# Ignaciagothe/tda-eeg-audio

Measured on AMD Instinct MI355X. Metric: windows/sec end-to-end (dist->Rips H0/H1->Wasserstein), 47-ch EEG, higher is better.
Workload: dtype f64; 1 GPU; configs[4]+configs[2]: 1416 recordings x 5 bands x 15 selected windows = 106200 (EEG 47x250 f64, audio 250 f64) window pairs per pass, the whole job; per pair corr->dist->Rips H0/H1 (EEG 47 pts), tau per recording-band, Takens dim 3 sub 2 + Rips (audio, 23..123 pts over the bands), Wasserstein H0+H1, features, per-recording reductions; one all-gather of the (1416, 5x48) rows per pass; windows_per_pass=106200, windows_per_gpu_per_pass=106200, input_bytes_per_gpu=10195200000, batches_per_pass=1, windows_per_batch=106200, parallelism=recordings dealt over 1 rank(s), one all-gather per pass, batches_in_flight=3, hip_graph=True, batches_rerun_with_full_ladder=0

## Files before the change

include/tdaeeg.h:

```cpp
#ifndef TDAEEG_H
#define TDAEEG_H

#include <stddef.h>

#ifdef __cplusplus
extern "C" {
#endif

typedef struct tda_ctx tda_ctx;

typedef enum {
    TDA_OK = 0,
    TDA_ERR_INVALID = 1,
    TDA_ERR_HIP = 2,
    TDA_ERR_UNSUPPORTED = 3,
    TDA_ERR_NOMEM = 4
} tda_status;

#define TDA_WIN_OK            0
#define TDA_WIN_H1_TRUNCATED  1
#define TDA_WIN_CLASS_OVERFLOW 2
#define TDA_WIN_DEGENERATE    4
#define TDA_WIN_NOT_CONVERGED 8
#define TDA_WIN_TOO_LARGE     16
// ... 125 lines not shown
tda_status tda_tau_segments_dev(tda_ctx* ctx, const double* win, const int* seg_off, int n_seg, int n_t,
                                int max_lag, int* tau_seg, int* tau_win, void* stream);

tda_status tda_features_batch_dev(tda_ctx* ctx, const double* dgm, const int* cnt, int n_dgm,
                                  int cap, double* feat, void* stream);
tda_status tda_features_batch(tda_ctx* ctx, const double* dgm, const int* cnt, int n_dgm,
                              int cap, double* feat);

typedef struct {
    double* rows;
    const int* cnt;
    int cap;
    int order;
    double* feat;
} tda_diagram_set;
tda_status tda_diagram_finish_dev(tda_ctx* ctx, const tda_diagram_set* sets, int n_sets, int n_dgm, void* stream);
#define TDA_ORDER_IN_CALL  0
#define TDA_ORDER_DEFERRED 1
tda_status tda_set_h1_order(tda_ctx* ctx, int policy);
#define TDA_SCHEME_LISTS 0
#define TDA_SCHEME_GRID  1
#define TDA_SCHEME_ONE   2
tda_status tda_set_launch_scheme(tda_ctx* ctx, int scheme);

tda_status tda_aggregate_batch_dev(tda_ctx* ctx, const double* feat_h0, const double* feat_h1,
                                   const int* seg_off, int n_seg, double* out, void* stream);
tda_status tda_aggregate_batch(tda_ctx* ctx, const double* feat_h0, const double* feat_h1,
                               const int* seg_off, int n_seg, int n_total, double* out);

tda_status tda_segment_nanmean_dev(tda_ctx* ctx, const double* x, const int* seg_off, int n_seg,
                                   double* out, void* stream);
tda_status tda_segment_nanmean(tda_ctx* ctx, const double* x, const int* seg_off, int n_seg,
                               int n_total, double* out);

tda_status tda_recording_rows_dev(tda_ctx* ctx, const double* w_h0, const double* w_h1, const int* tau_seg,
                                  const double* feat_h0, const double* feat_h1, const int* seg_off,
                                  int n_seg, double* out, const int* status_a, const int* status_b,
                                  int* seg_flags, void* stream);

tda_status tda_spearman_batch_dev(tda_ctx* ctx, const double* x, const double* y, int ld, const int* cols,
                                  int n_cols, const int* seg_off, int n_seg, double* r, void* stream);
tda_status tda_spearman_batch(tda_ctx* ctx, const double* x, const double* y, int n_total, int ld,
                              const int* cols, int n_cols, const int* seg_off, int n_seg, double* r);

tda_status tda_temporal_corr_dev(tda_ctx* ctx, const double* fa, const double* fe, int ld, const int* cols,
                                 int n_cols, const int* seg_off, int n_seg, const int* status_b, double* out,
// ... 50 lines not shown
```

tda_eeg_audio_amd/_lib.py:

```python
import contextlib
import ctypes as C
import os

import numpy as np

_HERE = os.path.dirname(os.path.abspath(__file__))
LIB_PATH = os.path.join(_HERE, os.path.basename(os.environ.get("TDA_LIB", "libtdaeeg.so")))

c_dp = C.POINTER(C.c_double)
c_ip = C.POINTER(C.c_int)
c_vp = C.c_void_p

TDA_WIN_H1_TRUNCATED = 1
TDA_WIN_CLASS_OVERFLOW = 2
TDA_WIN_DEGENERATE = 4
TDA_WIN_NOT_CONVERGED = 8
TDA_WIN_TOO_LARGE = 16
TDA_WIN_NO_PAIR = 32
N_FEATURES = 11
MAX_POINTS = 128

_I, _D = C.c_int, C.c_double
SYMBOLS = {
    "tda_version": (_I, []),
# ... 23 lines not shown
    "tda_sosfiltfilt": (_I, [c_vp, c_vp, _I, _I, c_vp, c_vp, _I, _I, c_vp]),
    "tda_filtfilt_dev": (_I, [c_vp, c_vp, _I, _I, c_vp, c_vp, c_vp, _I, _I, c_vp, c_vp, c_vp]),
    "tda_filtfilt": (_I, [c_vp, c_vp, _I, _I, c_vp, c_vp, c_vp, _I, _I, c_vp]),
    "tda_sosfiltfilt_bank_dev": (_I, [c_vp, c_vp, _I, _I, c_vp, c_vp, _I, _I, _I, c_vp, c_vp, c_vp]),
    "tda_filtfilt_bank_dev": (_I, [c_vp, c_vp, _I, _I, c_vp, c_vp, c_vp, _I, _I, _I, c_vp, c_vp, c_vp]),
    "tda_sosfiltfilt_bank_ragged_dev": (_I, [c_vp, c_vp, _I, _I, c_vp, c_vp, c_vp, c_vp, c_vp, _I, _I, _I, c_vp, c_vp, c_vp]),
    "tda_filtfilt_bank_ragged_dev": (_I, [c_vp, c_vp, _I, c_vp, c_vp, c_vp, c_vp, c_vp, c_vp, _I, _I, _I, c_vp, c_vp, c_vp]),
    "tda_gather_windows_dev": (_I, [c_vp, c_vp, c_vp, _I, _I, c_vp, c_vp]),
    "tda_eeg_window_ragged_dev": (_I, [c_vp, c_vp, c_vp, c_vp, _I, _I, _I, _D, c_vp, c_vp, c_vp, _I, c_vp, c_vp, _I, c_vp,
                                       c_vp, c_vp]),
    "tda_upfirdn_dev": (_I, [c_vp, c_vp, C.c_longlong, c_vp, _I, _I, _I, C.c_longlong, C.c_longlong, c_vp, c_vp]),
    "tda_upfirdn": (_I, [c_vp, c_vp, C.c_longlong, c_vp, _I, _I, _I, C.c_longlong, C.c_longlong, c_vp]),
    "tda_hilbert_envelope_dev": (_I, [c_vp, c_vp, _I, c_vp, c_vp, c_vp]),
    "tda_hilbert_envelope": (_I, [c_vp, c_vp, _I, c_vp, c_vp]),
    "tda_resample_poly_ragged_dev": (_I, [c_vp, c_vp, _I, c_vp, c_vp, c_vp, c_vp, c_vp, _I, _I, _I, _I, c_vp, c_vp]),
    "tda_hilbert_envelope_ragged_dev": (_I, [c_vp, c_vp, _I, c_vp, c_vp, c_vp, c_vp, c_vp, c_vp, c_vp]),
    "tda_tau_batch_dev": (_I, [c_vp, c_vp, _I, _I, _I, c_vp, c_vp]),
    "tda_tau_segments_dev": (_I, [c_vp, c_vp, c_vp, _I, _I, _I, c_vp, c_vp, c_vp]),
    "tda_recording_rows_dev": (_I, [c_vp, c_vp, c_vp, c_vp, c_vp, c_vp, c_vp, _I, c_vp, c_vp, c_vp, c_vp, c_vp]),
    "tda_set_retry_policy": (_I, [c_vp, _I]),
    "tda_set_retry_counter": (_I, [c_vp, c_vp]),
    "tda_set_h1_order": (_I, [c_vp, _I]),
    "tda_set_launch_scheme": (_I, [c_vp, _I]),
    "tda_diagram_finish_dev": (_I, [c_vp, c_vp, _I, _I, c_vp]),
    "tda_tau_batch": (_I, [c_vp, c_vp, _I, _I, _I, c_vp]),
    "tda_features_batch_dev": (_I, [c_vp, c_vp, c_vp, _I, _I, c_vp, c_vp]),
    "tda_features_batch": (_I, [c_vp, c_vp, c_vp, _I, _I, c_vp]),
    "tda_aggregate_batch_dev": (_I, [c_vp, c_vp, c_vp, c_vp, _I, c_vp, c_vp]),
    "tda_aggregate_batch": (_I, [c_vp, c_vp, c_vp, c_vp, _I, _I, c_vp]),
    "tda_segment_nanmean_dev": (_I, [c_vp, c_vp, c_vp, _I, c_vp, c_vp]),
    "tda_segment_nanmean": (_I, [c_vp, c_vp, c_vp, _I, _I, c_vp]),
    "tda_spearman_batch_dev": (_I, [c_vp, c_vp, c_vp, _I, c_vp, _I, c_vp, _I, c_vp, c_vp]),
    "tda_spearman_batch": (_I, [c_vp, c_vp, c_vp, _I, _I, c_vp, _I, c_vp, _I, c_vp]),
    "tda_temporal_corr_dev": (_I, [c_vp, c_vp, c_vp, _I, c_vp, _I, c_vp, _I, c_vp, c_vp, c_vp]),
    "tda_temporal_corr_batch": (_I, [c_vp, c_vp, c_vp, _I, _I, c_vp, _I, c_vp, _I, c_vp, c_vp]),
    "tda_wasserstein_batch_dev": (_I, [c_vp, c_vp, c_vp, _I, c_vp, c_vp, _I, c_vp, c_vp, _I, c_vp, c_vp, c_vp]),
    "tda_wasserstein_cross_dev": (_I, [c_vp, c_vp, c_vp, _I, _I, c_vp, c_vp, _I, c_vp, c_vp, _I, _I, c_vp, _I, c_vp, c_vp,
                                       c_vp, c_vp, c_vp]),
    "tda_cross_rows_dev": (_I, [c_vp, c_vp, c_vp, c_vp, c_vp, c_vp, _I, c_vp, c_vp, c_vp, c_vp]),
    "tda_wasserstein_matrix_dev": (_I, [c_vp, c_vp, c_vp, _I, _I, c_vp, _I, c_vp, c_vp, c_vp, _I, _I, c_vp, _I, _I, c_vp,
                                        c_vp, c_vp, c_vp, c_vp]),
    "tda_match_rows_dev": (_I, [c_vp, c_vp, c_vp, c_vp, _I, _I, c_vp, c_vp, c_vp, c_vp, c_vp, c_vp]),
    "tda_wasserstein_batch": (_I, [c_vp, c_vp, c_vp, _I, _I, c_vp, c_vp, _I, _I, c_vp, c_vp, _I, c_vp, c_vp]),
    "tda_event_create": (_I, [c_vp, C.POINTER(c_vp)]),
    "tda_event_record": (_I, [c_vp, c_vp, c_vp]),
    "tda_event_elapsed_ms": (_I, [c_vp, c_vp, c_vp, C.POINTER(C.c_float)]),
# ... 68 lines not shown

    ORDER_IN_CALL, ORDER_DEFERRED = 0, 1

    def set_h1_order(self, policy):
        self.check(self.lib.tda_set_h1_order(self.h, int(policy)))

    @contextlib.contextmanager
    def deferred(self, retry="auto"):
        if retry != "auto":
            self.set_retry_policy(self.RETRY_FIRST_PASS if retry == "first" else self.RETRY_ONE_STEP)
        self.set_h1_order(self.ORDER_DEFERRED)
        try:
            yield self
        finally:
            self.set_h1_order(self.ORDER_IN_CALL)
            if retry != "auto":
                self.set_retry_policy(self.RETRY_AUTO)

    SCHEME_LISTS, SCHEME_GRID, SCHEME_ONE = 0, 1, 2

    def set_launch_scheme(self, scheme):
        self.check(self.lib.tda_set_launch_scheme(self.h, int(scheme)))

    def set_retry_counter(self, dev_ptr):
        self.check(self.lib.tda_set_retry_counter(self.h, c_vp(dev_ptr) if dev_ptr else None))

    PROBES = {"rips_audio": 1, "rips_eeg": 2, "corr_dist": 3}

    def new_event(self):
        ev = c_vp()
        self.check(self.lib.tda_event_create(self.h, C.byref(ev)))
        return ev

    def arm_probe(self, stage, ev_start=None, ev_stop=None, dev_span=None):
        self.check(self.lib.tda_set_kernel_probe(self.h, self.PROBES[stage], ev_start, ev_stop,
                                                 c_vp(dev_span) if dev_span else None))

    def elapsed_ms(self, ev_start, ev_stop):
        ms = C.c_float()
        self.check(self.lib.tda_event_elapsed_ms(self.h, ev_start, ev_stop, C.byref(ms)))
        return float(ms.value)

    def close(self):
        if getattr(self, "h", None):
            self.lib.tda_ctx_destroy(self.h)
            self.h = None
# ... 39 lines not shown
```

tda_eeg_audio_amd/csrc/capi.hip:

```cpp
#include "common.h"
#include <string.h>
#include <vector>

static thread_local std::string g_create_err;

#pragma GCC visibility push(default)
extern "C" {

int tda_version(void) { return 100; }

tda_status tda_ctx_create(int device_id, tda_ctx** out)
{
    if (!out) return TDA_ERR_INVALID;
    *out = nullptr;
    int ndev = 0;
    hipError_t e = hipGetDeviceCount(&ndev);
    if (e != hipSuccess || ndev <= 0) {
        g_create_err = std::string("no HIP device: ") + hipGetErrorString(e);
        return TDA_ERR_HIP;
    }
    if (device_id < 0 || device_id >= ndev) { g_create_err = "device_id out of range"; return TDA_ERR_INVALID; }
    e = hipSetDevice(device_id);
    if (e != hipSuccess) { g_create_err = std::string("hipSetDevice: ") + hipGetErrorString(e); return TDA_ERR_HIP; }
    tda_ctx* c = new (std::nothrow) tda_ctx();
// ... 31 lines not shown
{
    if (!ctx) return TDA_ERR_INVALID;
    if ((words_dm != 0 && words_dm != 1 && words_dm != 2 && words_dm != 4) || (words_cloud != 1 && words_cloud != 2))
        TDA_FAIL(ctx, TDA_ERR_INVALID, "class words: dm in {0,1,2,4}, cloud in {1,2}");
    ctx->words_dm = words_dm;
    ctx->words_cloud = words_cloud;
    return TDA_OK;
}

tda_status tda_set_h1_order(tda_ctx* ctx, int policy)
{
    if (!ctx) return TDA_ERR_INVALID;
    if (policy != TDA_ORDER_IN_CALL && policy != TDA_ORDER_DEFERRED) TDA_FAIL(ctx, TDA_ERR_INVALID, "unknown order policy");
    ctx->h1_order = policy;
    return TDA_OK;
}

tda_status tda_set_launch_scheme(tda_ctx* ctx, int scheme)
{
    if (!ctx) return TDA_ERR_INVALID;
    if (scheme != TDA_SCHEME_LISTS && scheme != TDA_SCHEME_GRID && scheme != TDA_SCHEME_ONE)
        TDA_FAIL(ctx, TDA_ERR_INVALID, "unknown launch scheme");
    ctx->launch_scheme = scheme;
    return TDA_OK;
}

tda_status tda_diagram_finish_dev(tda_ctx* ctx, const tda_diagram_set* sets, int n_sets, int n_dgm, void* stream)
{
    if (!ctx) return TDA_ERR_INVALID;
    if (n_dgm < 0) TDA_FAIL(ctx, TDA_ERR_INVALID, "negative count");
    if (n_sets && !sets) TDA_FAIL(ctx, TDA_ERR_INVALID, "null pointer");
    return launch_diagram_finish(ctx, sets, n_sets, n_dgm, (hipStream_t)stream);
}

tda_status tda_set_retry_counter(tda_ctx* ctx, void* dev_counters)
{
    if (!ctx) return TDA_ERR_INVALID;
    ctx->retry_ctr = (unsigned long long*)dev_counters;
    return TDA_OK;
}

tda_status tda_set_retry_policy(tda_ctx* ctx, int policy)
{
    if (!ctx) return TDA_ERR_INVALID;
    if (policy < TDA_RETRY_AUTO || policy > TDA_RETRY_LAST_RUNG) TDA_FAIL(ctx, TDA_ERR_INVALID, "unknown retry policy");
    ctx->retry_policy = policy;
// ... 780 lines not shown
```

tda_eeg_audio_amd/csrc/common.h:

```cpp
#pragma once
#include <hip/hip_runtime.h>
#include <stdint.h>
#include <string>
#include <vector>
#include "../../include/tdaeeg.h"

typedef unsigned long long u64;
typedef uint32_t u32;
typedef uint16_t u16;

struct tda_ctx {
    int device = 0;
    int words_dm = 2;
    int words_cloud = 1;
    int retry_policy = 0;
    unsigned long long* retry_ctr = nullptr;
    unsigned long long* total_scratch = nullptr;
    int h1_order = 0;
    int launch_scheme = 0;
    int* retry_buf[32] = {};
    int* fin_list[32] = {};
    int* ws_list[32] = {};
    hipStream_t retry_stream[32] = {};
    int retry_streams = 0;
    int retry_shared = 0;
    int retry_cap = 0;
    std::vector<void*> retired;
    void* ws = nullptr;
    size_t ws_bytes = 0;
    std::string err;
    struct Probe { hipEvent_t start = nullptr, stop = nullptr; unsigned long long* span = nullptr; bool armed = false; };
    Probe probe[4];
};

struct ProbeScope {
    tda_ctx* ctx; hipStream_t st; int which; bool on; unsigned long long* span;
    ProbeScope(tda_ctx* c, int w, hipStream_t s)
        : ctx(c), st(s), which(w), on(w > 0 && w < 4 && c->probe[w].armed), span(nullptr)
    {
        if (on) {
            span = ctx->probe[which].span;
            if (ctx->probe[which].start) (void)hipEventRecord(ctx->probe[which].start, st);
// ... 172 lines not shown
```

tda_eeg_audio_amd/csrc/wasserstein.hip:

```cpp
#include "common.h"
#include <type_traits>

#ifdef TDA_PROFILE
__device__ unsigned long long g_prof_ws[16];
extern "C" __attribute__((visibility("default"))) int tda_profile_read_ws(unsigned long long* out, int reset)
{
    if (hipMemcpyFromSymbol(out, HIP_SYMBOL(g_prof_ws), sizeof(unsigned long long) * 16) != hipSuccess) return 1;
    if (reset) {
        unsigned long long z[16] = {0};
        if (hipMemcpyToSymbol(HIP_SYMBOL(g_prof_ws), z, sizeof(z)) != hipSuccess) return 1;
    }
    return 0;
}
#define WPROF(i, v) do { if (lane_id() == 0) atomicAdd(&g_prof_ws[i], (unsigned long long)(v)); } while (0)
#define WCLK() clock64()
#else
#define WPROF(i, v) do {} while (0)
#define WCLK() 0ull
#endif

#define WS_DEFERRED 0x40000000
#define WS_CP 0.7071067811865476
#define WS_SP 0.7071067811865475

// ... 5 lines not shown
}

__device__ __forceinline__ double wave_min_f64_ws(double v)
{
#pragma unroll
    for (int off = 32; off > 0; off >>= 1) {
        const double o = __shfl_xor(v, off, 64);
        v = o < v ? o : v;
    }
    return v;
}

__device__ __forceinline__ double ws_cost(double ab, double ad, double bb, double bd)
{
    const double xx = ab * ab + ad * ad;
    const double yy = bb * bb + bd * bd;
    const double dot = fma(ad, bd, ab * bb);
    double d2 = -2.0 * dot;
    d2 += xx;
    d2 += yy;
    if (!(d2 > 0.0)) d2 = 0.0;
    return sqrt_rn(d2);
}

struct ws_index_pairs {
    const int* idx_a; const int* idx_b;
    __device__ __forceinline__ bool resolve(int pr, int& ia, int& ib) const
    {
        ia = idx_a ? idx_a[pr] : pr;
        ib = idx_b ? idx_b[pr] : pr;
        return true;
    }
};
struct ws_table_pairs {
    const int* grp_a; const int* seg_off_a; const int* seg_off_b; const int* partner_seg; const int* status_b;
    int n_seg_a, n_seg_b, n_b;
    __device__ __forceinline__ bool resolve(int pr, int& ia, int& ib) const
    {
        ia = pr;
        const int g = grp_a[pr];
        if (g < 0 || g >= n_seg_a) return false;
        const int p = partner_seg[g];
        if (p < 0 || p >= n_seg_b) return false;
        const int i = pr - seg_off_a[g];
        const int b0 = seg_off_b[p];
        if (i < 0 || i >= seg_off_b[p + 1] - b0) return false;
        ib = b0 + i;
        if (ib < 0 || ib >= n_b) return false;
        return !(status_b[ib] & TDA_WIN_DEGENERATE);
    }
};

struct ws_matrix_pairs {
    const int* status_b; int a0, b0, len_b, n_b;
    __device__ __forceinline__ bool resolve(int pr, int& ia, int& ib) const
    {
        ia = a0 + pr;
        if (pr >= len_b) return false;
        ib = b0 + pr;
        if (ib < 0 || ib >= n_b) return false;
        return !(status_b[ib] & TDA_WIN_DEGENERATE);
    }
};

template <int CW, class SRC>
__device__ __forceinline__ void ws_solve(const double* __restrict__ dgm_a, const int* __restrict__ cnt_a, int cap_a,
                                         const double* __restrict__ dgm_b, const int* __restrict__ cnt_b, int cap_b,
                                         const SRC& src, int pr, int max_rows, int max_cols,
                                         double* __restrict__ out, int* __restrict__ status, int mode, int* list,
                                         unsigned char* smem)
{
    const int lane = lane_id();
    unsigned long long wt0 = WCLK();
    (void)wt0;
    double* rb = reinterpret_cast<double*>(smem);
    double* rd = rb + max_rows;
    double* rs = rd + max_rows;
    double* ru = rs + max_rows;
    double* cb = ru + max_rows;
    double* cd = cb + max_cols;
    double* ct = cd + max_cols;
    int* owner = reinterpret_cast<int*>(ct + max_cols);
    double* G = ct + max_cols + ((max_cols + 1) >> 1);

    int ia, ib;
    if (!src.resolve(pr, ia, ib)) {
        if (lane == 0) { out[pr] = __longlong_as_double(0x7ff8000000000000ll); status[pr] = TDA_WIN_NO_PAIR; }
        return;
    }
    const double* A = dgm_a + (size_t)ia * cap_a * 2;
    const double* B = dgm_b + (size_t)ib * cap_b * 2;
    int ka = cnt_a[ia]; ka = ka < cap_a ? ka : cap_a; ka = ka < 0 ? 0 : ka;
    int kb = cnt_b[ib]; kb = kb < cap_b ? kb : cap_b; kb = kb < 0 ? 0 : kb;
// ... 41 lines not shown
            const int i = i0 + lane;
            double b = 0, d = 0; bool fin = false;
            if (i < kb) { b = B[2 * i]; d = B[2 * i + 1]; fin = isfinite(b) && isfinite(d); }
            const u64 bal = __ballot(fin);
            const int pos = m + __popcll(bal & ((1ull << lane) - 1ull));
            if (fin) { pb[pos] = b; pd[pos] = d; pc[pos] = fma(d, WS_CP, -(b * WS_SP)); }
            m += __popcll(bal);
        }
        if (N == 0 && lane == 0) { pb[0] = 0.0; pd[0] = 0.0; pc[0] = 0.0; }
    }
    __syncthreads();

    auto cfull = [&](int i, int j) -> double {
        return a_is_row ? ws_cost(rb[i], rd[i], cb[j], cd[j]) : ws_cost(cb[j], cd[j], rb[i], rd[i]);
    };
    auto gain = [&](int i, int j) -> double {
        const double g = cfull(i, j) - rs[i] - ct[j];
        return g < 0.0 ? g : 0.0;
    };
    for (int i = lane; i < R; i += 64) ru[i] = 0.0;
    __syncthreads();
    WPROF(0, WCLK() - wt0); wt0 = WCLK();
    WPROF(4, 1); WPROF(5, R); WPROF(6, Cn);

    {
        bool ok = R <= 64;
        const double b0 = rb[0];
        for (int i0 = 0; i0 < R; i0 += 64) {
            const int i = i0 + lane;
            ok = ok && !__ballot(i < R && (rb[i] != b0 || (i + 1 < R && rd[i + 1] < rd[i])));
        }
        for (int j0 = 0; j0 < Cn; j0 += 64) {
            const int j = j0 + lane;
            ok = ok && !__ballot(j < Cn && (cb[j] != b0 || (j + 1 < Cn && cd[j + 1] < cd[j])));
        }
        if (ok) {
            double cur = 0.0, nb1 = 0.0, nb2 = 0.0;
            const int nsteps1d = R + Cn - 1;
            for (int j = lane; j < Cn; j += 64) G[j] = cb[j] * cb[j] + cd[j] * cd[j];
            __syncthreads();
            const int li = lane < R ? lane : 0;
            const double r_b = rb[li], r_d = rd[li], r_s = rs[li], r_n = r_b * r_b + r_d * r_d;
            const double bb = b0 * b0;
            auto wavefront = [&](auto AROW) {
                constexpr bool A_ROW = decltype(AROW)::value;
                for (int t = 0; t < nsteps1d; ++t) {
                    const int j0 = t - lane;
                    const int lo = __builtin_amdgcn_update_dpp(0, __double2loint(cur), 0x138, 0xF, 0xF, false);
                    const int hi = __builtin_amdgcn_update_dpp(0, __double2hiint(cur), 0x138, 0xF, 0xF, false);
                    nb2 = nb1;
                    nb1 = __hiloint2double(hi, lo);
                    if (lane < R && j0 >= 0 && j0 < Cn) {
                        const double c_d = cd[j0], c_n = G[j0];
                        const double dot = fma(r_d, c_d, bb);
                        double d2 = -2.0 * dot;
                        d2 += A_ROW ? r_n : c_n;
                        d2 += A_ROW ? c_n : r_n;
                        if (!(d2 > 0.0)) d2 = 0.0;
                        double g = sqrt_rn(d2) - r_s - ct[j0];
                        g = g < 0.0 ? g : 0.0;
                        const double up = nb1;
                        const double dg = (j0 == 0 ? 0.0 : nb2) + g;
                        double m = up < cur ? up : cur;
                        m = dg < m ? dg : m;
                        cur = m;
                    }
                }
            };
            if (a_is_row) wavefront(std::true_type{}); else wavefront(std::false_type{});
            const double fbest = uni_f64(cur, R - 1);
            double part = 0.0;
            for (int i = lane; i < R; i += 64) part += rs[i];
            for (int j = lane; j < Cn; j += 64) part += ct[j];
            const double total1d = wave_sum_f64(part) + fbest;
            if (lane == 0) { out[pr] = total1d; status[pr] = 0; }
            return;
        }
    }

    double v[CW], minv[CW], u[CW];
    int prow[CW], way[CW];
    bool used[CW], rowin[CW];
#pragma unroll
    for (int c = 0; c < CW; ++c) { v[c] = 0.0; u[c] = 0.0; prow[c] = -1; way[c] = -1; }

    const double INF = __longlong_as_double(0x7ff0000000000000ll);
    bool failed = false;
    int nsteps = 0;
    (void)nsteps;
    bool rowdone[CW];
    {
        int myarg[CW];
        for (int j = lane; j < Cn; j += 64) owner[j] = 0x7fffffff;
        __syncthreads();
#pragma unroll
        for (int c = 0; c < CW; ++c) {
            const int r = lane + 64 * c;
            myarg[c] = -1; rowdone[c] = false;
            if (c < cw_used && r < R) {
                double mn = INF; int arg = 0;
                int j = r < Cn ? r : 0;
#pragma unroll 4
                for (int t = 0; t < Cn; ++t) {
                    const double g = gain(r, j);
                    if (g < mn) { mn = g; arg = j; }
                    j = (j + 1 == Cn) ? 0 : j + 1;
                }
                u[c] = mn; myarg[c] = arg;
                atomicMin(&owner[arg], r);
            }
        }
        __syncthreads();
#pragma unroll
        for (int c = 0; c < CW; ++c) {
            if (myarg[c] >= 0) rowdone[c] = owner[myarg[c]] == lane + 64 * c;
            const int j = lane + 64 * c;
            if (c < cw_used && j < Cn) { const int o = owner[j]; prow[c] = (o != 0x7fffffff) ? o : -1; }
        }
    }
    for (int i = 0; i < R && !failed; ++i) {
        {
            int dn = 0;
#pragma unroll
            for (int c = 0; c < CW; ++c)
                if (c == (i >> 6)) dn = (int)rl32((u32)(rowdone[c] ? 1 : 0), i & 63);
            if (dn) continue;
        }
#pragma unroll
        for (int c = 0; c < CW; ++c) { minv[c] = INF; used[c] = false; rowin[c] = (lane + 64 * c) == i; }
        int i0 = i, j0 = -1;
        int steps = 0;
        while (true) {
            double ui0 = 0.0;
#pragma unroll
            for (int c = 0; c < CW; ++c)
                if (c == (i0 >> 6)) ui0 = uni_f64(u[c], i0 & 63);
            double best = INF, gg[CW];
#pragma unroll
            for (int c = 0; c < CW; ++c) {
                if (c >= cw_used) break;
                const int j = lane + 64 * c;
                const int jc = j < Cn ? j : Cn - 1;
                gg[c] = gain(i0, jc);
// ... 49 lines not shown
        if (failed) break;
        int guard = 0;
        while (j0 >= 0 && guard++ < Cn + 2) {
            const int c0 = j0 >> 6, l0 = j0 & 63;
            int jprev = -1;
#pragma unroll
            for (int c = 0; c < CW; ++c)
                if (c == c0) jprev = (int)rl32((u32)way[c], l0);
            int newrow = i;
            if (jprev >= 0) {
                const int cp = jprev >> 6, lp = jprev & 63;
#pragma unroll
                for (int c = 0; c < CW; ++c)
                    if (c == cp) newrow = (int)rl32((u32)prow[c], lp);
            }
#pragma unroll
            for (int c = 0; c < CW; ++c)
                if (c == c0 && lane == l0) prow[c] = newrow;
            j0 = jprev;
        }
    }
    if (failed) {
        if (lane == 0) { out[pr] = __longlong_as_double(0x7ff8000000000000ll); status[pr] = TDA_WIN_NOT_CONVERGED; }
        return;
    }
    WPROF(1, WCLK() - wt0); wt0 = WCLK();
    WPROF(3, nsteps);
    double part = 0.0;
    __syncthreads();
    for (int i = lane; i < R; i += 64) ru[i] = 0.0;
    __syncthreads();
#pragma unroll
    for (int c = 0; c < CW; ++c) {
        const int j = lane + 64 * c;
        if (j < Cn) {
            bool real = false;
            if (prow[c] >= 0) {
                const double cf = cfull(prow[c], j);
                if (cf - rs[prow[c]] - ct[j] < 0.0) { real = true; part += cf; ru[prow[c]] = 1.0; }
            }
            if (!real) part += ct[j];
        }
    }
    __syncthreads();
    for (int i = lane; i < R; i += 64)
        if (ru[i] == 0.0) part += rs[i];
    const double total = wave_sum_f64(part);
    if (lane == 0) { out[pr] = total; status[pr] = 0; }
    WPROF(2, WCLK() - wt0);
}

template <int CW, class SRC>
__global__ void __launch_bounds__(64)
wasserstein_kernel(const double* __restrict__ dgm_a, const int* __restrict__ cnt_a, int cap_a,
                   const double* __restrict__ dgm_b, const int* __restrict__ cnt_b, int cap_b,
                   const SRC src, int n_pairs,
                   int max_rows, int max_cols,
                   double* __restrict__ out, int* __restrict__ status, int mode, int* list)
{
    extern __shared__ __attribute__((aligned(16))) unsigned char smem[];
    const int pr = blockIdx.x;
    if (pr >= n_pairs) return;
    if (mode == 2 && status[pr] != WS_DEFERRED) return;
    ws_solve<CW, SRC>(dgm_a, cnt_a, cap_a, dgm_b, cnt_b, cap_b, src, pr, max_rows, max_cols, out, status, mode, list, smem);
}

template <int CW, class SRC>
__global__ void __launch_bounds__(64)
wasserstein_list_kernel(const double* __restrict__ dgm_a, const int* __restrict__ cnt_a, int cap_a,
                        const double* __restrict__ dgm_b, const int* __restrict__ cnt_b, int cap_b,
                        const SRC src, int n_pairs,
                        int max_rows, int max_cols,
                        double* __restrict__ out, int* __restrict__ status, int* list)
{
    extern __shared__ __attribute__((aligned(16))) unsigned char smem[];
    int nl = uni(list[0]);
    nl = nl < n_pairs ? nl : n_pairs;
    for (int j = blockIdx.x; j < nl; j += gridDim.x) {
        const int pr = uni(list[4 + j]);
        if (pr >= 0 && pr < n_pairs)
            ws_solve<CW, SRC>(dgm_a, cnt_a, cap_a, dgm_b, cnt_b, cap_b, src, pr, max_rows, max_cols, out, status, 0, nullptr, smem);
        __syncthreads();
    }
    if (threadIdx.x == 0 && atomicAdd(&list[1], 1) == (int)gridDim.x - 1) { list[0] = 0; list[1] = 0; }
}

template <class SRC>
static tda_status launch_wasserstein_src(tda_ctx* ctx, const double* dgm_a, const int* cnt_a, int cap_a, const double* dgm_b,
                                         const int* cnt_b, int cap_b, const SRC& src, int n_pairs, double* out, int* status,
                                         hipStream_t st)
{
    if (n_pairs == 0) return TDA_OK;
    if (cap_a < 1 || cap_b < 1) TDA_FAIL(ctx, TDA_ERR_INVALID, "diagram capacity must be >= 1");
    const int lo = cap_a < cap_b ? cap_a : cap_b, hi = cap_a < cap_b ? cap_b : cap_a;
    const int max_rows = lo, max_cols = hi;
    if (max_cols > 512) TDA_FAIL(ctx, TDA_ERR_UNSUPPORTED, "diagrams with more than 512 rows are not supported");
    const size_t lds = (size_t)(4 * max_rows + 4 * max_cols + ((max_cols + 1) >> 1)) * 8;
    static const bool one_launch = getenv("TDA_WS_ONE_LAUNCH") != nullptr;
    const int scheme = one_launch ? TDA_SCHEME_ONE : ctx->launch_scheme;
    const int mode = (scheme != TDA_SCHEME_ONE && max_cols > 128) ? 2 : 0;
    int* list = nullptr;
    if (mode && scheme == TDA_SCHEME_LISTS) {
        int slot = -1;
        const tda_status rc = stream_lists_take(ctx, n_pairs, st, &slot);
        if (rc != TDA_OK) return rc;
        if (slot >= 0) list = ctx->ws_list[slot];
    }
    if (mode) {
        const int sr = max_rows < 64 ? max_rows : 64;
        const size_t lds_s = (size_t)(4 * sr + 4 * 64 + 32) * 8;
        hipLaunchKernelGGL((wasserstein_kernel<1, SRC>), dim3(n_pairs), dim3(64), lds_s, st, dgm_a, cnt_a, cap_a, dgm_b, cnt_b,
                           cap_b, src, n_pairs, sr, 64, out, status, 1, list);
    }
#define WS_LAUNCH(CWV)                                                                                         \
    do {                                                                                                       \
        auto kern = wasserstein_kernel<CWV, SRC>;                                                              \
        auto lkern = wasserstein_list_kernel<CWV, SRC>;                                                        \
        if (lds > 48 * 1024)                                                                                   \
            TDA_HIP(ctx, hipFuncSetAttribute(list ? reinterpret_cast<const void*>(lkern)                       \
                                                  : reinterpret_cast<const void*>(kern),                       \
                                             hipFuncAttributeMaxDynamicSharedMemorySize, (int)lds));           \
        if (list)                                                                                              \
            hipLaunchKernelGGL(lkern, dim3(n_pairs < 256 ? n_pairs : 256), dim3(64), lds, st, dgm_a, cnt_a,    \
                               cap_a, dgm_b, cnt_b, cap_b, src, n_pairs, max_rows, max_cols, out, status, list); \
        else                                                                                                   \
            hipLaunchKernelGGL(kern, dim3(n_pairs), dim3(64), lds, st, dgm_a, cnt_a, cap_a, dgm_b, cnt_b,      \
                               cap_b, src, n_pairs, max_rows, max_cols, out, status, mode, (int*)nullptr);     \
    } while (0)
    if (max_cols <= 128) WS_LAUNCH(2);
    else if (max_cols <= 256) WS_LAUNCH(4);
    else WS_LAUNCH(8);
#undef WS_LAUNCH
    TDA_HIP(ctx, hipGetLastError());
    return TDA_OK;
}

tda_status launch_wasserstein(tda_ctx* ctx, const double* dgm_a, const int* cnt_a, int cap_a, const double* dgm_b,
                              const int* cnt_b, int cap_b, const int* idx_a, const int* idx_b, int n_pairs,
                              double* out, int* status, hipStream_t st)
{
    return launch_wasserstein_src(ctx, dgm_a, cnt_a, cap_a, dgm_b, cnt_b, cap_b, ws_index_pairs{idx_a, idx_b}, n_pairs, out,
                                  status, st);
}

tda_status launch_wasserstein_cross(tda_ctx* ctx, const double* dgm_a, const int* cnt_a, int cap_a, int n_a,
                                    const int* grp_a, const int* seg_off_a, int n_seg_a, const double* dgm_b,
                                    const int* cnt_b, int cap_b, int n_b, const int* seg_off_b, int n_seg_b,
                                    const int* status_b, const int* partner_seg, double* out, int* status, hipStream_t st)
{
    const ws_table_pairs src{grp_a, seg_off_a, seg_off_b, partner_seg, status_b, n_seg_a, n_seg_b, n_b};
// ... 10 lines not shown
template <class F>
__device__ __forceinline__ double ws_np_sum(const F& f, int n)
{
    if (n < 8) {
        double res = 0.0;
        for (int i = 0; i < n; ++i) res += f(i);
        return res;
    }
    double r0 = f(0), r1 = f(1), r2 = f(2), r3 = f(3), r4 = f(4), r5 = f(5), r6 = f(6), r7 = f(7);
    int i;
    for (i = 8; i < n - (n % 8); i += 8) {
        r0 += f(i + 0); r1 += f(i + 1); r2 += f(i + 2); r3 += f(i + 3);
        r4 += f(i + 4); r5 += f(i + 5); r6 += f(i + 6); r7 += f(i + 7);
    }
    double res = ((r0 + r1) + (r2 + r3)) + ((r4 + r5) + (r6 + r7));
    for (; i < n; ++i) res += f(i);
    return res;
}

template <int CW>
__device__ __forceinline__ void ws_matrix_entry(const double* __restrict__ dgm_a, const int* __restrict__ cnt_a, int cap_a,
                                                const double* __restrict__ dgm_b, const int* __restrict__ cnt_b, int cap_b,
                                                const ws_matrix_args& M, size_t e, int e_rel, int max_rows, int max_cols,
                                                int solver_bytes, int mode, int* list, unsigned char* smem)
{
    const int lane = lane_id();
    const double qnan = __longlong_as_double(0x7ff8000000000000ll);
    const int g = (int)(e / (size_t)M.n_col), c = (int)(e % (size_t)M.n_col);
    const int a0 = uni(M.seg_off_a[g]), a1 = uni(M.seg_off_a[g + 1]);
    const int len = (a0 >= 0 && a1 >= a0 && a1 <= M.n_a) ? a1 - a0 : 0;
    const int k = uni(M.cls_a[g]);
    int b0 = 0, len_b = 0;
    if (k >= 0 && k < M.n_cls) {
        const size_t p = (size_t)k * M.n_col + c;
        b0 = uni(M.seg_off_b[p]);
        len_b = uni(M.seg_off_b[p + 1]) - b0;
    }
    if (len > WS_MATRIX_MAX_GROUP) {
        if (lane == 0) { M.out[e] = qnan; M.pairs[e] = 0; M.flags[e] = TDA_WIN_TOO_LARGE; }
        return;
    }
    double* xs = reinterpret_cast<double*>(smem + solver_bytes);
    int* ss = reinterpret_cast<int*>(xs + WS_MATRIX_MAX_GROUP);
    const ws_matrix_pairs src{M.status_b, a0, b0, len_b, M.n_b};
    const int n_try = len < len_b ? len : len_b;
    if (lane >= n_try && lane < len) { xs[lane] = qnan; ss[lane] = TDA_WIN_NO_PAIR; }
    bool deferred = false;
    for (int i = 0; i < n_try && !deferred; ++i) {
        ws_solve<CW>(dgm_a, cnt_a, cap_a, dgm_b, cnt_b, cap_b, src, i, max_rows, max_cols, xs, ss, mode ? 1 : 0, nullptr, smem);
        __syncthreads();
        deferred = mode && uni(ss[i]) == WS_DEFERRED;
    }
    if (deferred) {
        if (lane == 0) {
            if (list) list[4 + atomicAdd(&list[0], 1)] = e_rel;
            else M.flags[e] = WS_DEFERRED;
        }
        return;
    }
    __syncthreads();
    if (lane == 0) {
        int n = 0, cnt = 0, fl = 0;
        for (int i = 0; i < len; ++i) n += (ss[i] & TDA_WIN_NO_PAIR) ? 0 : 1;
        for (int i = 0; i < n; ++i) {
            cnt += (ss[i] == 0 && xs[i] == xs[i]) ? 1 : 0;
            fl |= ss[i];
        }
        auto val = [=](int j) { const double v = xs[j]; return (ss[j] == 0 && v == v) ? v : 0.0; };
        const double sum = ws_np_sum(val, n);
        M.out[e] = cnt > 0 ? sum / (double)cnt : qnan;
        M.pairs[e] = n;
        M.flags[e] = fl & ~(TDA_WIN_NO_PAIR | TDA_WIN_DEGENERATE);
    }
}

template <int CW>
__global__ void __launch_bounds__(64)
wasserstein_matrix_kernel(const double* __restrict__ dgm_a, const int* __restrict__ cnt_a, int cap_a,
                          const double* __restrict__ dgm_b, const int* __restrict__ cnt_b, int cap_b,
                          const ws_matrix_args M, size_t e0, int n_e, int max_rows, int max_cols, int solver_bytes, int mode,
                          int* list)
{
    extern __shared__ __attribute__((aligned(16))) unsigned char smem[];
    if ((int)blockIdx.x >= n_e) return;
    const size_t e = e0 + blockIdx.x;
    if (mode == 2 && M.flags[e] != WS_DEFERRED) return;
    ws_matrix_entry<CW>(dgm_a, cnt_a, cap_a, dgm_b, cnt_b, cap_b, M, e, (int)blockIdx.x, max_rows, max_cols, solver_bytes,
                        mode == 1, list, smem);
}

template <int CW>
__global__ void __launch_bounds__(64)
wasserstein_matrix_list_kernel(const double* __restrict__ dgm_a, const int* __restrict__ cnt_a, int cap_a,
                               const double* __restrict__ dgm_b, const int* __restrict__ cnt_b, int cap_b,
                               const ws_matrix_args M, size_t e0, int n_e, int max_rows, int max_cols, int solver_bytes,
                               int* list)
{
    extern __shared__ __attribute__((aligned(16))) unsigned char smem[];
    int nl = uni(list[0]);
    nl = nl < n_e ? nl : n_e;
    for (int j = blockIdx.x; j < nl; j += gridDim.x) {
        const int r = uni(list[4 + j]);
        if (r >= 0 && r < n_e)
            ws_matrix_entry<CW>(dgm_a, cnt_a, cap_a, dgm_b, cnt_b, cap_b, M, e0 + (size_t)r, r, max_rows, max_cols, solver_bytes, 0,
                                nullptr, smem);
        __syncthreads();
    }
    if (threadIdx.x == 0 && atomicAdd(&list[1], 1) == (int)gridDim.x - 1) { list[0] = 0; list[1] = 0; }
}

#define WS_MATRIX_CHUNK (1 << 16)
#define WS_MATRIX_GRID_CHUNK (1 << 30)
#define WS_MATRIX_LIST_GRID 2048

tda_status launch_wasserstein_matrix(tda_ctx* ctx, const double* dgm_a, const int* cnt_a, int cap_a, int n_a,
                                     const int* seg_off_a, int n_seg_a, const int* cls_a, const double* dgm_b,
                                     const int* cnt_b, int cap_b, int n_b, const int* seg_off_b, int n_cls, int n_col,
                                     const int* status_b, double* out, int* pairs, int* flags, hipStream_t st)
{
    const size_t n_ent = (size_t)n_seg_a * (size_t)n_col;
    if (n_ent == 0) return TDA_OK;
    if (cap_a < 1 || cap_b < 1) TDA_FAIL(ctx, TDA_ERR_INVALID, "diagram capacity must be >= 1");
    const int lo = cap_a < cap_b ? cap_a : cap_b, hi = cap_a < cap_b ? cap_b : cap_a;
    const int max_rows = lo, max_cols = hi;
    if (max_cols > 512) TDA_FAIL(ctx, TDA_ERR_UNSUPPORTED, "diagrams with more than 512 rows are not supported");
    const ws_matrix_args M{seg_off_a, cls_a, seg_off_b, status_b, n_a, n_b, n_cls, n_col, out, pairs, flags};
    const size_t lds_res = (size_t)WS_MATRIX_MAX_GROUP * 12;
    const int lds_solver = (4 * max_rows + 4 * max_cols + ((max_cols + 1) >> 1)) * 8;
    const size_t lds_w = lds_solver + lds_res;
    const int sr = max_rows < 64 ? max_rows : 64;
    const int lds_solver_s = (4 * sr + 4 * 64 + 32) * 8;
    const size_t lds_s = lds_solver_s + lds_res;
    static const bool one_launch = getenv("TDA_WS_ONE_LAUNCH") != nullptr;
    const int scheme = one_launch ? TDA_SCHEME_ONE : ctx->launch_scheme;
    const int mode = (scheme != TDA_SCHEME_ONE && max_cols > 128) ? 2 : 0;
    int* list = nullptr;
    if (mode && scheme == TDA_SCHEME_LISTS) {
        int slot = -1;
        const tda_status rc = stream_lists_take(ctx, (int)(n_ent < WS_MATRIX_CHUNK ? n_ent : WS_MATRIX_CHUNK), st, &slot);
        if (rc != TDA_OK) return rc;
        if (slot >= 0) list = ctx->ws_list[slot];
    }
    const size_t chunk = list ? WS_MATRIX_CHUNK : WS_MATRIX_GRID_CHUNK;
    for (size_t e0 = 0; e0 < n_ent; e0 += chunk) {
        const int n_e = (int)(n_ent - e0 < chunk ? n_ent - e0 : chunk);
        if (mode)
            hipLaunchKernelGGL(wasserstein_matrix_kernel<1>, dim3(n_e), dim3(64), lds_s, st, dgm_a, cnt_a, cap_a, dgm_b, cnt_b,
                               cap_b, M, e0, n_e, sr, 64, lds_solver_s, 1, list);
#define WS_MATRIX_LAUNCH(CWV)                                                                                  \
    do {                                                                                                       \
        auto kern = wasserstein_matrix_kernel<CWV>;                                                            \
        auto lkern = wasserstein_matrix_list_kernel<CWV>;                                                      \
        if (lds_w > 48 * 1024)                                                                                 \
            TDA_HIP(ctx, hipFuncSetAttribute(list ? reinterpret_cast<const void*>(lkern)                       \
                                                  : reinterpret_cast<const void*>(kern),                       \
                                             hipFuncAttributeMaxDynamicSharedMemorySize, (int)lds_w));         \
        if (list)                                                                                              \
            hipLaunchKernelGGL(lkern, dim3(n_e < WS_MATRIX_LIST_GRID ? n_e : WS_MATRIX_LIST_GRID), dim3(64), lds_w, st,  \
                               dgm_a, cnt_a, cap_a, dgm_b, cnt_b, cap_b, M, e0, n_e, max_rows, max_cols, lds_solver, list); \
        else                                                                                                   \
            hipLaunchKernelGGL(kern, dim3(n_e), dim3(64), lds_w, st, dgm_a, cnt_a, cap_a, dgm_b, cnt_b, cap_b, \
                               M, e0, n_e, max_rows, max_cols, lds_solver, mode, (int*)nullptr);               \
    } while (0)
        if (max_cols <= 128) WS_MATRIX_LAUNCH(2);
        else if (max_cols <= 256) WS_MATRIX_LAUNCH(4);
        else WS_MATRIX_LAUNCH(8);
#undef WS_MATRIX_LAUNCH
    }
    TDA_HIP(ctx, hipGetLastError());
    return TDA_OK;
}
```

Before: 4.254 million windows/s.

## Prune Wasserstein solver: trim dead rows/cols in 1D path, skip all-diagonal assignments

Adds geometric pruning to the Wasserstein solver, enabled by default. In the 1D fast path it drops leading and trailing rows and columns whose points can never beat their diagonal cost, which shortens the wavefront. In the general path it computes bounding boxes and skips the whole assignment when no row can match any column cheaper than the diagonal. The bounds use a relative-plus-absolute margin, so results should stay exact. In exchange it adds reduction work per pair, an optional atomic counter, and a new API setter to turn pruning off.

```diff
diff --git a/include/tdaeeg.h b/include/tdaeeg.h
--- a/include/tdaeeg.h
+++ b/include/tdaeeg.h
@@ -171,6 +171,8 @@
 #define TDA_SCHEME_GRID  1
 #define TDA_SCHEME_ONE   2
 tda_status tda_set_launch_scheme(tda_ctx* ctx, int scheme);
+tda_status tda_set_wasserstein_pruning(tda_ctx* ctx, int on);
+tda_status tda_set_wasserstein_counter(tda_ctx* ctx, unsigned long long* dev_counters);
 
 tda_status tda_aggregate_batch_dev(tda_ctx* ctx, const double* feat_h0, const double* feat_h1,
                                    const int* seg_off, int n_seg, double* out, void* stream);
diff --git a/tda_eeg_audio_amd/_lib.py b/tda_eeg_audio_amd/_lib.py
--- a/tda_eeg_audio_amd/_lib.py
+++ b/tda_eeg_audio_amd/_lib.py
@@ -69,6 +69,8 @@
     "tda_set_retry_counter": (_I, [c_vp, c_vp]),
     "tda_set_h1_order": (_I, [c_vp, _I]),
     "tda_set_launch_scheme": (_I, [c_vp, _I]),
+    "tda_set_wasserstein_pruning": (_I, [c_vp, _I]),
+    "tda_set_wasserstein_counter": (_I, [c_vp, c_vp]),
     "tda_diagram_finish_dev": (_I, [c_vp, c_vp, _I, _I, c_vp]),
     "tda_tau_batch": (_I, [c_vp, c_vp, _I, _I, _I, c_vp]),
     "tda_features_batch_dev": (_I, [c_vp, c_vp, c_vp, _I, _I, c_vp, c_vp]),
@@ -183,6 +185,12 @@
     def set_launch_scheme(self, scheme):
         self.check(self.lib.tda_set_launch_scheme(self.h, int(scheme)))
 
+    def set_wasserstein_pruning(self, on=True):
+        self.check(self.lib.tda_set_wasserstein_pruning(self.h, 1 if on else 0))
+
+    def set_wasserstein_counter(self, dev_ptr):
+        self.check(self.lib.tda_set_wasserstein_counter(self.h, c_vp(dev_ptr) if dev_ptr else None))
+
     def set_retry_counter(self, dev_ptr):
         self.check(self.lib.tda_set_retry_counter(self.h, c_vp(dev_ptr) if dev_ptr else None))
 
diff --git a/tda_eeg_audio_amd/csrc/capi.hip b/tda_eeg_audio_amd/csrc/capi.hip
--- a/tda_eeg_audio_amd/csrc/capi.hip
+++ b/tda_eeg_audio_amd/csrc/capi.hip
@@ -77,6 +77,20 @@
     if (scheme != TDA_SCHEME_LISTS && scheme != TDA_SCHEME_GRID && scheme != TDA_SCHEME_ONE)
         TDA_FAIL(ctx, TDA_ERR_INVALID, "unknown launch scheme");
     ctx->launch_scheme = scheme;
+    return TDA_OK;
+}
+
+tda_status tda_set_wasserstein_pruning(tda_ctx* ctx, int on)
+{
+    if (!ctx) return TDA_ERR_INVALID;
+    ctx->ws_prune = on ? 1 : 0;
+    return TDA_OK;
+}
+
+tda_status tda_set_wasserstein_counter(tda_ctx* ctx, unsigned long long* dev_counters)
+{
+    if (!ctx) return TDA_ERR_INVALID;
+    ctx->ws_ctr = dev_counters;
     return TDA_OK;
 }
 
diff --git a/tda_eeg_audio_amd/csrc/common.h b/tda_eeg_audio_amd/csrc/common.h
--- a/tda_eeg_audio_amd/csrc/common.h
+++ b/tda_eeg_audio_amd/csrc/common.h
@@ -18,6 +18,8 @@
     unsigned long long* total_scratch = nullptr;
     int h1_order = 0;
     int launch_scheme = 0;
+    int ws_prune = 1;
+    unsigned long long* ws_ctr = nullptr;
     int* retry_buf[32] = {};
     int* fin_list[32] = {};
     int* ws_list[32] = {};
diff --git a/tda_eeg_audio_amd/csrc/wasserstein.hip b/tda_eeg_audio_amd/csrc/wasserstein.hip
--- a/tda_eeg_audio_amd/csrc/wasserstein.hip
+++ b/tda_eeg_audio_amd/csrc/wasserstein.hip
@@ -51,6 +51,15 @@
     if (!(d2 > 0.0)) d2 = 0.0;
     return sqrt_rn(d2);
 }
+
+struct ws_opts {
+    unsigned long long* ctr;
+    int prune;
+};
+
+#define WS_PRUNE_REL 1e-6
+#define WS_PRUNE_ABS 1e-150
+#define WS_PRUNE_MAX 1e150
 
 struct ws_index_pairs {
     const int* idx_a; const int* idx_b;
@@ -97,7 +106,7 @@
                                          const double* __restrict__ dgm_b, const int* __restrict__ cnt_b, int cap_b,
                                          const SRC& src, int pr, int max_rows, int max_cols,
                                          double* __restrict__ out, int* __restrict__ status, int mode, int* list,
-                                         unsigned char* smem)
+                                         const ws_opts& opt, unsigned char* smem)
 {
     const int lane = lane_id();
     unsigned long long wt0 = WCLK();
@@ -185,6 +194,14 @@
     __syncthreads();
     WPROF(0, WCLK() - wt0); wt0 = WCLK();
     WPROF(4, 1); WPROF(5, R); WPROF(6, Cn);
+    unsigned long long n_cut = 0, n_trim = 0;
+    auto count = [&]() {
+        if (opt.ctr && lane == 0) {
+            if (n_cut) atomicAdd(&opt.ctr[0], n_cut);
+            if (n_trim) atomicAdd(&opt.ctr[1], n_trim);
+            atomicAdd(&opt.ctr[2], 1ull);
+        }
+    };
 
     {
         bool ok = R <= 64;
@@ -198,11 +215,42 @@
             ok = ok && !__ballot(j < Cn && (cb[j] != b0 || (j + 1 < Cn && cd[j + 1] < cd[j])));
         }
         if (ok) {
+            int ilo = 0, jlo = 0, Rl = R, Cl = Cn;
+            const double c1p = 1.0 + WS_CP, c1m = 1.0 - WS_CP;
+            double mx = WS_PRUNE_MAX;
+            if (opt.prune)
+                mx = fmax(fabs(b0), fmax(fmax(fabs(rd[0]), fabs(rd[R - 1])), fmax(fabs(cd[0]), fabs(cd[Cn - 1]))));
+            if (mx < WS_PRUNE_MAX) {
+                const double p_min = rd[0] - b0, p_max = rd[R - 1] - b0;
+                const double m = WS_PRUNE_REL * mx + WS_PRUNE_ABS;
+                const double lo_c = p_min * c1m - m, hi_c = p_max * c1p + m;
+                int n_lo = 0, n_hi = 0;
+                for (int j0 = 0; j0 < Cn; j0 += 64) {
+                    const int j = j0 + lane;
+                    const double q = cd[j < Cn ? j : Cn - 1] - b0;
+                    n_lo += __popcll(__ballot(j < Cn && q * c1p <= lo_c));
+                    n_hi += __popcll(__ballot(j < Cn && q * c1m >= hi_c));
+                }
+                jlo = n_lo;
+                const int jhi = Cn - n_hi > jlo ? Cn - n_hi : jlo;
+                Cl = jhi - jlo;
+                Rl = 0;
+                if (Cl > 0) {
+                    const double q_min = cd[jlo] - b0, q_max = cd[jhi - 1] - b0;
+                    const double lo_r = q_min * c1m - m, hi_r = q_max * c1p + m;
+                    const double p = rd[lane < R ? lane : R - 1] - b0;
+                    ilo = __popcll(__ballot(lane < R && p * c1p <= lo_r));
+                    const int ihi = R - __popcll(__ballot(lane < R && p * c1m >= hi_r));
+                    Rl = ihi > ilo ? ihi - ilo : 0;
+                }
+                n_trim = (unsigned long long)((R - Rl) + (Cn - Cl));
+            }
+            WPROF(8, 1); WPROF(9, Rl); WPROF(10, Cl);
             double cur = 0.0, nb1 = 0.0, nb2 = 0.0;
-            const int nsteps1d = R + Cn - 1;
+            const int nsteps1d = (Rl > 0 && Cl > 0) ? Rl + Cl - 1 : 0;
             for (int j = lane; j < Cn; j += 64) G[j] = cb[j] * cb[j] + cd[j] * cd[j];
             __syncthreads();
-            const int li = lane < R ? lane : 0;
+            const int li = lane < Rl ? ilo + lane : 0;
             const double r_b = rb[li], r_d = rd[li], r_s = rs[li], r_n = r_b * r_b + r_d * r_d;
             const double bb = b0 * b0;
             auto wavefront = [&](auto AROW) {
@@ -213,14 +261,14 @@
                     const int hi = __builtin_amdgcn_update_dpp(0, __double2hiint(cur), 0x138, 0xF, 0xF, false);
                     nb2 = nb1;
                     nb1 = __hiloint2double(hi, lo);
-                    if (lane < R && j0 >= 0 && j0 < Cn) {
-                        const double c_d = cd[j0], c_n = G[j0];
+                    if (lane < Rl && j0 >= 0 && j0 < Cl) {
+                        const double c_d = cd[jlo + j0], c_n = G[jlo + j0];
                         const double dot = fma(r_d, c_d, bb);
                         double d2 = -2.0 * dot;
                         d2 += A_ROW ? r_n : c_n;
                         d2 += A_ROW ? c_n : r_n;
                         if (!(d2 > 0.0)) d2 = 0.0;
-                        double g = sqrt_rn(d2) - r_s - ct[j0];
+                        double g = sqrt_rn(d2) - r_s - ct[jlo + j0];
                         g = g < 0.0 ? g : 0.0;
                         const double up = nb1;
                         const double dg = (j0 == 0 ? 0.0 : nb2) + g;
@@ -231,15 +279,58 @@
                 }
             };
             if (a_is_row) wavefront(std::true_type{}); else wavefront(std::false_type{});
-            const double fbest = uni_f64(cur, R - 1);
+            const double fbest = nsteps1d ? uni_f64(cur, Rl - 1) : 0.0;
             double part = 0.0;
             for (int i = lane; i < R; i += 64) part += rs[i];
             for (int j = lane; j < Cn; j += 64) part += ct[j];
             const double total1d = wave_sum_f64(part) + fbest;
             if (lane == 0) { out[pr] = total1d; status[pr] = 0; }
+            count();
             return;
         }
     }
+
+    bool all_dead = false;
+    if (opt.prune) {
+        const double INFP = __longlong_as_double(0x7ff0000000000000ll);
+        double rb_lo = INFP, rb_hi = -INFP, rd_lo = INFP, rd_hi = -INFP, s_hi = -INFP;
+        double cb_lo = INFP, cb_hi = -INFP, cd_lo = INFP, cd_hi = -INFP, t_hi = -INFP;
+        for (int i = lane; i < R; i += 64) {
+            rb_lo = fmin(rb_lo, rb[i]); rb_hi = fmax(rb_hi, rb[i]);
+            rd_lo = fmin(rd_lo, rd[i]); rd_hi = fmax(rd_hi, rd[i]);
+            s_hi = fmax(s_hi, rs[i]);
+        }
+        for (int j = lane; j < Cn; j += 64) {
+            cb_lo = fmin(cb_lo, cb[j]); cb_hi = fmax(cb_hi, cb[j]);
+            cd_lo = fmin(cd_lo, cd[j]); cd_hi = fmax(cd_hi, cd[j]);
+            t_hi = fmax(t_hi, ct[j]);
+        }
+        rb_lo = wave_min_f64_dpp(rb_lo); rb_hi = wave_max_f64_dpp(rb_hi);
+        rd_lo = wave_min_f64_dpp(rd_lo); rd_hi = wave_max_f64_dpp(rd_hi);
+        cb_lo = wave_min_f64_dpp(cb_lo); cb_hi = wave_max_f64_dpp(cb_hi);
+        cd_lo = wave_min_f64_dpp(cd_lo); cd_hi = wave_max_f64_dpp(cd_hi);
+        s_hi = wave_max_f64_dpp(s_hi); t_hi = wave_max_f64_dpp(t_hi);
+        const double mx = fmax(fmax(fmax(fabs(rb_lo), fabs(rb_hi)), fmax(fabs(rd_lo), fabs(rd_hi))),
+                               fmax(fmax(fabs(cb_lo), fabs(cb_hi)), fmax(fabs(cd_lo), fabs(cd_hi))));
+        if (mx < WS_PRUNE_MAX) {
+            const double m = WS_PRUNE_REL * mx + WS_PRUNE_ABS;
+            const double gx = fmax(0.0, fmax(cb_lo - rb_hi, rb_lo - cb_hi));
+            const double gy = fmax(0.0, fmax(cd_lo - rd_hi, rd_lo - cd_hi));
+            all_dead = sqrt_rn(gx * gx + gy * gy) > s_hi + t_hi + m;
+            if (!all_dead) {
+                bool live = false;
+                for (int i0 = 0; i0 < R; i0 += 64) {
+                    const int i = i0 + lane < R ? i0 + lane : R - 1;
+                    const double dx = fmax(0.0, fmax(cb_lo - rb[i], rb[i] - cb_hi));
+                    const double dy = fmax(0.0, fmax(cd_lo - rd[i], rd[i] - cd_hi));
+                    live = live || __ballot(!(sqrt_rn(dx * dx + dy * dy) > rs[i] + t_hi + m)) != 0ull;
+                }
+                all_dead = !live;
+            }
+        }
+        if (all_dead) n_cut = 1;
+    }
+    WPROF(7, all_dead ? 1 : 0);
 
     double v[CW], minv[CW], u[CW];
     int prow[CW], way[CW];
@@ -252,7 +343,7 @@
     int nsteps = 0;
     (void)nsteps;
     bool rowdone[CW];
-    {
+    if (!all_dead) {
         int myarg[CW];
         for (int j = lane; j < Cn; j += 64) owner[j] = 0x7fffffff;
         __syncthreads();
@@ -281,7 +372,7 @@
             if (c < cw_used && j < Cn) { const int o = owner[j]; prow[c] = (o != 0x7fffffff) ? o : -1; }
         }
     }
-    for (int i = 0; i < R && !failed; ++i) {
+    for (int i = 0; i < R && !failed && !all_dead; ++i) {
         {
             int dn = 0;
 #pragma unroll
@@ -377,6 +468,7 @@
     }
     if (failed) {
         if (lane == 0) { out[pr] = __longlong_as_double(0x7ff8000000000000ll); status[pr] = TDA_WIN_NOT_CONVERGED; }
+        count();
         return;
     }
     WPROF(1, WCLK() - wt0); wt0 = WCLK();
@@ -402,6 +494,7 @@
         if (ru[i] == 0.0) part += rs[i];
     const double total = wave_sum_f64(part);
     if (lane == 0) { out[pr] = total; status[pr] = 0; }
+    count();
     WPROF(2, WCLK() - wt0);
 }
 
@@ -411,13 +504,13 @@
                    const double* __restrict__ dgm_b, const int* __restrict__ cnt_b, int cap_b,
                    const SRC src, int n_pairs,
                    int max_rows, int max_cols,
-                   double* __restrict__ out, int* __restrict__ status, int mode, int* list)
+                   double* __restrict__ out, int* __restrict__ status, int mode, int* list, const ws_opts opt)
 {
     extern __shared__ __attribute__((aligned(16))) unsigned char smem[];
     const int pr = blockIdx.x;
     if (pr >= n_pairs) return;
     if (mode == 2 && status[pr] != WS_DEFERRED) return;
-    ws_solve<CW, SRC>(dgm_a, cnt_a, cap_a, dgm_b, cnt_b, cap_b, src, pr, max_rows, max_cols, out, status, mode, list, smem);
+    ws_solve<CW, SRC>(dgm_a, cnt_a, cap_a, dgm_b, cnt_b, cap_b, src, pr, max_rows, max_cols, out, status, mode, list, opt, smem);
 }
 
 template <int CW, class SRC>
@@ -426,7 +519,7 @@
                         const double* __restrict__ dgm_b, const int* __restrict__ cnt_b, int cap_b,
                         const SRC src, int n_pairs,
                         int max_rows, int max_cols,
-                        double* __restrict__ out, int* __restrict__ status, int* list)
+                        double* __restrict__ out, int* __restrict__ status, int* list, const ws_opts opt)
 {
     extern __shared__ __attribute__((aligned(16))) unsigned char smem[];
     int nl = uni(list[0]);
@@ -434,7 +527,7 @@
     for (int j = blockIdx.x; j < nl; j += gridDim.x) {
         const int pr = uni(list[4 + j]);
         if (pr >= 0 && pr < n_pairs)
-            ws_solve<CW, SRC>(dgm_a, cnt_a, cap_a, dgm_b, cnt_b, cap_b, src, pr, max_rows, max_cols, out, status, 0, nullptr, smem);
+            ws_solve<CW, SRC>(dgm_a, cnt_a, cap_a, dgm_b, cnt_b, cap_b, src, pr, max_rows, max_cols, out, status, 0, nullptr, opt, smem);
         __syncthreads();
     }
     if (threadIdx.x == 0 && atomicAdd(&list[1], 1) == (int)gridDim.x - 1) { list[0] = 0; list[1] = 0; }
@@ -449,6 +542,7 @@
     if (cap_a < 1 || cap_b < 1) TDA_FAIL(ctx, TDA_ERR_INVALID, "diagram capacity must be >= 1");
     const int lo = cap_a < cap_b ? cap_a : cap_b, hi = cap_a < cap_b ? cap_b : cap_a;
     const int max_rows = lo, max_cols = hi;
+    const ws_opts opt{ctx->ws_ctr, ctx->ws_prune};
     if (max_cols > 512) TDA_FAIL(ctx, TDA_ERR_UNSUPPORTED, "diagrams with more than 512 rows are not supported");
     const size_t lds = (size_t)(4 * max_rows + 4 * max_cols + ((max_cols + 1) >> 1)) * 8;
     static const bool one_launch = getenv("TDA_WS_ONE_LAUNCH") != nullptr;
@@ -465,7 +559,7 @@
         const int sr = max_rows < 64 ? max_rows : 64;
         const size_t lds_s = (size_t)(4 * sr + 4 * 64 + 32) * 8;
         hipLaunchKernelGGL((wasserstein_kernel<1, SRC>), dim3(n_pairs), dim3(64), lds_s, st, dgm_a, cnt_a, cap_a, dgm_b, cnt_b,
-                           cap_b, src, n_pairs, sr, 64, out, status, 1, list);
+                           cap_b, src, n_pairs, sr, 64, out, status, 1, list, opt);
     }
 #define WS_LAUNCH(CWV)                                                                                         \
     do {                                                                                                       \
@@ -477,10 +571,10 @@
                                              hipFuncAttributeMaxDynamicSharedMemorySize, (int)lds));           \
         if (list)                                                                                              \
             hipLaunchKernelGGL(lkern, dim3(n_pairs < 256 ? n_pairs : 256), dim3(64), lds, st, dgm_a, cnt_a,    \
-                               cap_a, dgm_b, cnt_b, cap_b, src, n_pairs, max_rows, max_cols, out, status, list); \
+                               cap_a, dgm_b, cnt_b, cap_b, src, n_pairs, max_rows, max_cols, out, status, list, opt); \
         else                                                                                                   \
             hipLaunchKernelGGL(kern, dim3(n_pairs), dim3(64), lds, st, dgm_a, cnt_a, cap_a, dgm_b, cnt_b,      \
-                               cap_b, src, n_pairs, max_rows, max_cols, out, status, mode, (int*)nullptr);     \
+                               cap_b, src, n_pairs, max_rows, max_cols, out, status, mode, (int*)nullptr, opt); \
     } while (0)
     if (max_cols <= 128) WS_LAUNCH(2);
     else if (max_cols <= 256) WS_LAUNCH(4);
@@ -537,7 +631,8 @@
 __device__ __forceinline__ void ws_matrix_entry(const double* __restrict__ dgm_a, const int* __restrict__ cnt_a, int cap_a,
                                                 const double* __restrict__ dgm_b, const int* __restrict__ cnt_b, int cap_b,
                                                 const ws_matrix_args& M, size_t e, int e_rel, int max_rows, int max_cols,
-                                                int solver_bytes, int mode, int* list, unsigned char* smem)
+                                                int solver_bytes, int mode, int* list, const ws_opts& opt,
+                                                unsigned char* smem)
 {
     const int lane = lane_id();
     const double qnan = __longlong_as_double(0x7ff8000000000000ll);
@@ -562,7 +657,7 @@
     if (lane >= n_try && lane < len) { xs[lane] = qnan; ss[lane] = TDA_WIN_NO_PAIR; }
     bool deferred = false;
     for (int i = 0; i < n_try && !deferred; ++i) {
-        ws_solve<CW>(dgm_a, cnt_a, cap_a, dgm_b, cnt_b, cap_b, src, i, max_rows, max_cols, xs, ss, mode ? 1 : 0, nullptr, smem);
+        ws_solve<CW>(dgm_a, cnt_a, cap_a, dgm_b, cnt_b, cap_b, src, i, max_rows, max_cols, xs, ss, mode ? 1 : 0, nullptr, opt, smem);
         __syncthreads();
         deferred = mode && uni(ss[i]) == WS_DEFERRED;
     }
@@ -594,14 +689,14 @@
 wasserstein_matrix_kernel(const double* __restrict__ dgm_a, const int* __restrict__ cnt_a, int cap_a,
                           const double* __restrict__ dgm_b, const int* __restrict__ cnt_b, int cap_b,
                           const ws_matrix_args M, size_t e0, int n_e, int max_rows, int max_cols, int solver_bytes, int mode,
-                          int* list)
+                          int* list, const ws_opts opt)
 {
     extern __shared__ __attribute__((aligned(16))) unsigned char smem[];
     if ((int)blockIdx.x >= n_e) return;
     const size_t e = e0 + blockIdx.x;
     if (mode == 2 && M.flags[e] != WS_DEFERRED) return;
     ws_matrix_entry<CW>(dgm_a, cnt_a, cap_a, dgm_b, cnt_b, cap_b, M, e, (int)blockIdx.x, max_rows, max_cols, solver_bytes,
-                        mode == 1, list, smem);
+                        mode == 1, list, opt, smem);
 }
 
 template <int CW>
@@ -609,7 +704,7 @@
 wasserstein_matrix_list_kernel(const double* __restrict__ dgm_a, const int* __restrict__ cnt_a, int cap_a,
                                const double* __restrict__ dgm_b, const int* __restrict__ cnt_b, int cap_b,
                                const ws_matrix_args M, size_t e0, int n_e, int max_rows, int max_cols, int solver_bytes,
-                               int* list)
+                               int* list, const ws_opts opt)
 {
     extern __shared__ __attribute__((aligned(16))) unsigned char smem[];
     int nl = uni(list[0]);
@@ -618,7 +713,7 @@
         const int r = uni(list[4 + j]);
         if (r >= 0 && r < n_e)
             ws_matrix_entry<CW>(dgm_a, cnt_a, cap_a, dgm_b, cnt_b, cap_b, M, e0 + (size_t)r, r, max_rows, max_cols, solver_bytes, 0,
-                                nullptr, smem);
+                                nullptr, opt, smem);
         __syncthreads();
     }
     if (threadIdx.x == 0 && atomicAdd(&list[1], 1) == (int)gridDim.x - 1) { list[0] = 0; list[1] = 0; }
@@ -640,6 +735,7 @@
     const int max_rows = lo, max_cols = hi;
     if (max_cols > 512) TDA_FAIL(ctx, TDA_ERR_UNSUPPORTED, "diagrams with more than 512 rows are not supported");
     const ws_matrix_args M{seg_off_a, cls_a, seg_off_b, status_b, n_a, n_b, n_cls, n_col, out, pairs, flags};
+    const ws_opts opt{ctx->ws_ctr, ctx->ws_prune};
     const size_t lds_res = (size_t)WS_MATRIX_MAX_GROUP * 12;
     const int lds_solver = (4 * max_rows + 4 * max_cols + ((max_cols + 1) >> 1)) * 8;
     const size_t lds_w = lds_solver + lds_res;
@@ -661,7 +757,7 @@
         const int n_e = (int)(n_ent - e0 < chunk ? n_ent - e0 : chunk);
         if (mode)
             hipLaunchKernelGGL(wasserstein_matrix_kernel<1>, dim3(n_e), dim3(64), lds_s, st, dgm_a, cnt_a, cap_a, dgm_b, cnt_b,
-                               cap_b, M, e0, n_e, sr, 64, lds_solver_s, 1, list);
+                               cap_b, M, e0, n_e, sr, 64, lds_solver_s, 1, list, opt);
 #define WS_MATRIX_LAUNCH(CWV)                                                                                  \
     do {                                                                                                       \
         auto kern = wasserstein_matrix_kernel<CWV>;                                                            \
@@ -672,10 +768,10 @@
                                              hipFuncAttributeMaxDynamicSharedMemorySize, (int)lds_w));         \
         if (list)                                                                                              \
             hipLaunchKernelGGL(lkern, dim3(n_e < WS_MATRIX_LIST_GRID ? n_e : WS_MATRIX_LIST_GRID), dim3(64), lds_w, st,  \
-                               dgm_a, cnt_a, cap_a, dgm_b, cnt_b, cap_b, M, e0, n_e, max_rows, max_cols, lds_solver, list); \
+                               dgm_a, cnt_a, cap_a, dgm_b, cnt_b, cap_b, M, e0, n_e, max_rows, max_cols, lds_solver, list, opt); \
         else                                                                                                   \
             hipLaunchKernelGGL(kern, dim3(n_e), dim3(64), lds_w, st, dgm_a, cnt_a, cap_a, dgm_b, cnt_b, cap_b, \
-                               M, e0, n_e, max_rows, max_cols, lds_solver, mode, (int*)nullptr);               \
+                               M, e0, n_e, max_rows, max_cols, lds_solver, mode, (int*)nullptr, opt);          \
     } while (0)
         if (max_cols <= 128) WS_MATRIX_LAUNCH(2);
         else if (max_cols <= 256) WS_MATRIX_LAUNCH(4);
```

Measured after the change: 4.392 million windows/s, median of 6. +3.2%, better.
